# andrewjong/SwapNet

Measured on NVIDIA H100. Metric: images/sec (G+D fwd+bwd) warp-stage 512x512, higher is better.
Workload: dtype fp16/bf16-split x3 tensor-core products, fp32 accumulate (fp32-faithful)

## Files before the change

include/swapnet_b200.h:

```cpp
#ifndef SWAPNET_B200_H
#define SWAPNET_B200_H

#include <stdint.h>

#ifdef __cplusplus
extern "C" {
#endif

#define SN_MAX_TAPS 32
#define SN_MAX_SRC 3

enum { SN_ACT_NONE = 0, SN_ACT_TANH = 1, SN_ACT_LRELU = 2, SN_ACT_RELU = 3 };
enum { SN_LAYOUT_NCHW = 0, SN_LAYOUT_NHWC = 1, SN_LAYOUT_LABEL_U8 = 2, SN_LAYOUT_MASK_I32 = 3 };
#define SN_FMT_BF16 0
#define SN_FMT_F16 1

const char* sn_version(void);
const char* sn_last_error(void);
long long sn_launch_count(void);
void sn_count_replayed(long long n);

typedef struct sn_tap {
  int c_off;
  int kb_off;
// ... 43 lines not shown
  int ksplit;
  int nsplit;
  int deterministic;
} sn_wgrad_desc;

typedef struct sn_plan sn_plan;

int sn_tap_gemm_plan_create(const sn_tap_gemm_desc* desc, sn_plan** out);
int sn_wgrad_plan_create(const sn_wgrad_desc* desc, sn_plan** out);
int sn_plan_run(const sn_plan* plan, void* stream);
void sn_plan_destroy(sn_plan* plan);
int sn_plan_has_stats(const sn_plan* plan);
int sn_plan_geometry(const sn_plan* plan, int* out);
long long sn_plan_workspace_bytes(const sn_plan* plan);
int sn_wgrad_ksplit(const sn_wgrad_desc* desc, int sm_count);

int sn_pack_planes(const float* src, int src_layout, int src_pitch, int n, int c, int h, int w,
                   void* dst_hi, void* dst_lo, int dst_pitch, int dst_coff, int fmt, void* stream);

int sn_pack_concat(int lead, const float* src0, int layout0, int pitch0, int c0, const float* src1, int layout1,
                   int pitch1, int c1, int n, int h, int w, int c_fill, void* dst_hi, void* dst_lo, void* dst2_hi,
                   void* dst2_lo, int dst_pitch, int dst_coff, int fmt, int fmt2, void* stream);

typedef struct sn_scale_item { const float* w; long long count; float* scale2; } sn_scale_item;
typedef struct sn_pack_item {
  const float* src; long long s_row, s_k;
  int rows, taps, taps_pitch, k_real, k_pad, fmt;
  void* hi; void* lo; const float* scale2;
  int slot[16];
  int block_begin;
// ... 224 lines not shown
```

swapnet_b200/_lib.py:

```python
from __future__ import annotations

import ctypes as C
import os

_HERE = os.path.dirname(os.path.abspath(__file__))
LIB_PATH = os.path.join(_HERE, "libswapnet_b200.so")

SN_MAX_TAPS = 32
SN_MAX_SRC = 3
ACT_NONE, ACT_TANH, ACT_LRELU, ACT_RELU = 0, 1, 2, 3
LAYOUT_NCHW, LAYOUT_NHWC, LAYOUT_LABEL_U8, LAYOUT_MASK_I32 = 0, 1, 2, 3
FMT_BF16, FMT_F16 = 0, 1
AUG_NONE, AUG_HFLIP, AUG_VFLIP, AUG_AFFINE_NEAREST, AUG_PERSPECTIVE_BILINEAR = 0, 1, 2, 3, 4
AUG_MAX_OPS = 8


class SnTap(C.Structure):
    _fields_ = [("c_off", C.c_int), ("kb_off", C.c_int), ("dw", C.c_int), ("dh", C.c_int), ("hp", C.c_int)]


class SnTapGemmDesc(C.Structure):
    _fields_ = [
        ("a_hi", C.c_void_p), ("a_lo", C.c_void_p),
        ("a_n", C.c_int), ("a_h", C.c_int), ("a_w", C.c_int), ("a_c", C.c_int), ("a_pitch", C.c_int),
# ... 100 lines not shown

_VP, _I, _LL, _F, _ULL = C.c_void_p, C.c_int, C.c_longlong, C.c_float, C.c_ulonglong
SIGNATURES = {
    "sn_version": (C.c_char_p, []),
    "sn_last_error": (C.c_char_p, []),
    "sn_launch_count": (_LL, []),
    "sn_count_replayed": (None, [_LL]),
    "sn_tap_gemm_plan_create": (_I, [C.POINTER(SnTapGemmDesc), C.POINTER(_VP)]),
    "sn_wgrad_plan_create": (_I, [C.POINTER(SnWgradDesc), C.POINTER(_VP)]),
    "sn_plan_run": (_I, [_VP, _VP]),
    "sn_plan_destroy": (None, [_VP]),
    "sn_plan_has_stats": (_I, [_VP]),
    "sn_plan_geometry": (_I, [_VP, C.POINTER(C.c_int)]),
    "sn_plan_workspace_bytes": (_LL, [_VP]),
    "sn_wgrad_ksplit": (_I, [C.POINTER(SnWgradDesc), _I]),
    "sn_det_slots": (_LL, [_I, _I]),
    "sn_plane_sums_det": (_I, [_VP, _I, _I, _I, _I, _VP, _VP, _LL, _VP]),
    "sn_plane_stats_det": (_I, [_VP, _I, _I, _I, _I, _F, _VP, _VP, _LL, _VP]),
    "sn_bias_grad_det": (_I, [_VP, _VP, _I, _I, _I, _LL, _I, _VP, _VP, _VP, _LL, _VP]),
    "sn_ce_tanh_bwd_det": (_I, [_VP, _I, _VP, _I, C.POINTER(SnGradSrc), _I, _I, _I, _I, _I, _F, _VP, _VP, _VP, _I, _I,
                                _I, _VP, _LL, _VP]),
    "sn_gan_loss_fwd_bwd_det": (_I, [_I, _VP, _LL, _I, _F, _F, _VP, _F, _VP, _VP, _VP, _LL, _VP]),
    "sn_l1_loss_fwd_bwd_det": (_I, [_VP, _I, _VP, _I, _I, _I, _I, _F, _VP, _VP, _I, _VP, _LL, _VP]),
    "sn_to_one_wgrad_det": (_I, [_VP, _VP, _I, _I, _I, _I, _I, _I, _VP, _VP, _I, _I, _I, _I, _VP, _VP, _LL, _VP]),
    "sn_to_one_wgrad_det_slots": (_LL, [_I]),
    "sn_stats_finalize": (_I, [_VP, _I, _I, _F, _VP]),
    "sn_plane_sums": (_I, [_VP, _I, _I, _I, _I, _VP, _VP]),
    "sn_bn_finalize": (_I, [_VP, _I, _I, _I, _I, _F, _F, _VP, _VP, _VP, _VP]),
    "sn_bn_eval_stats": (_I, [_VP, _I, _I, _VP, _VP, _F, _VP]),
    "sn_bn_group_sums": (_I, [_VP, _I, _I, _I, _I, _VP, _VP]),
# ... 91 lines not shown
```

swapnet_b200/csrc/api.cu:

```cuda
#include <stdarg.h>
#include <atomic>
#include "common.cuh"
#include "plan.h"

static thread_local char g_err[1024] = "";
std::atomic<long long> g_launches{0};

void sn_set_error(const char* fmt, ...) {
  va_list ap;
  va_start(ap, fmt);
  vsnprintf(g_err, sizeof(g_err), fmt, ap);
  va_end(ap);
}
void sn_count_launch(int n) { g_launches.fetch_add(n, std::memory_order_relaxed); }

struct sn_plan {
  int kind;
  TapGemmPlan tg;
  WgradPlan wg;
};

static int g_sm_count = 0;
static int sm_count() {
  if (!g_sm_count) {
// ... 53 lines not shown
  out[0] = plan->kind;
  out[1] = (int)g.x;
  out[2] = (int)g.y;
  out[3] = (int)g.z;
  out[4] = plan->kind == 0 ? plan->tg.p.block_n : plan->wg.p.block_n;
  out[5] = plan->kind == 0 ? plan->tg.p.a_chunk : plan->wg.p.y_chunk;
  return SN_OK;
}

long long sn_plan_workspace_bytes(const sn_plan* plan) {
  return plan && plan->kind == 1 ? (long long)plan->wg.ws_bytes : 0;
}

int sn_wgrad_ksplit(const sn_wgrad_desc* desc, int sm_count) { return sn_wgrad_plan_ksplit(desc, sm_count); }

void sn_plan_destroy(sn_plan* plan) {
  if (plan && plan->kind == 0 && plan->tg.p.tile_counter) cudaFree(plan->tg.p.tile_counter);
  if (plan && plan->kind == 1 && plan->wg.p.det_ws) cudaFree(plan->wg.p.det_ws);
  delete plan;
}

}
```

swapnet_b200/csrc/common.cuh:

```cuda
#pragma once
#include <cuda_runtime.h>
#include <cuda.h>
#include <cuda_bf16.h>
#include <cuda_fp16.h>
#include <stdint.h>
#include <stdio.h>
#include <string.h>

void sn_set_error(const char* fmt, ...);
#define SN_OK 0
#define SN_ERR_INVALID (-1)
#define SN_ERR_CUDA (-2)
#define SN_ERR_UNSUPPORTED (-3)
#define SN_NUM_SMS 132
#ifndef SN_FMT_BF16
#define SN_FMT_BF16 0
#define SN_FMT_F16 1
#endif

#define SN_CHECK_CUDA(expr)                                                        \
  do {                                                                             \
    cudaError_t _e = (expr);                                                       \
    if (_e != cudaSuccess) {                                                       \
      sn_set_error("%s:%d CUDA error %s: %s", __FILE__, __LINE__, #expr,           \
// ... 203 lines not shown
        "{\n.reg .pred p;\nsetp.ne.b32 p, %66, 0;\n"
        "wgmma.mma_async.sync.aligned.m64n128k16.f32.bf16.bf16 "
        "{%0, %1, %2, %3, %4, %5, %6, %7, %8, %9, %10, %11, %12, %13, %14, %15, %16, %17, %18, %19, %20, %21, %22, %23, %24, %25, %26, %27, %28, %29, %30, %31, %32, %33, %34, %35, %36, %37, %38, %39, %40, %41, %42, %43, %44, %45, %46, %47, %48, %49, %50, %51, %52, %53, %54, %55, %56, %57, %58, %59, %60, %61, %62, %63}, %64, %65, p, 1, 1, %67, %68;\n}\n"
        : "+f"(d[0]), "+f"(d[1]), "+f"(d[2]), "+f"(d[3]), "+f"(d[4]), "+f"(d[5]), "+f"(d[6]), "+f"(d[7]), "+f"(d[8]), "+f"(d[9]), "+f"(d[10]), "+f"(d[11]), "+f"(d[12]), "+f"(d[13]), "+f"(d[14]), "+f"(d[15]), "+f"(d[16]), "+f"(d[17]), "+f"(d[18]), "+f"(d[19]), "+f"(d[20]), "+f"(d[21]), "+f"(d[22]), "+f"(d[23]), "+f"(d[24]), "+f"(d[25]), "+f"(d[26]), "+f"(d[27]), "+f"(d[28]), "+f"(d[29]), "+f"(d[30]), "+f"(d[31]), "+f"(d[32]), "+f"(d[33]), "+f"(d[34]), "+f"(d[35]), "+f"(d[36]), "+f"(d[37]), "+f"(d[38]), "+f"(d[39]), "+f"(d[40]), "+f"(d[41]), "+f"(d[42]), "+f"(d[43]), "+f"(d[44]), "+f"(d[45]), "+f"(d[46]), "+f"(d[47]), "+f"(d[48]), "+f"(d[49]), "+f"(d[50]), "+f"(d[51]), "+f"(d[52]), "+f"(d[53]), "+f"(d[54]), "+f"(d[55]), "+f"(d[56]), "+f"(d[57]), "+f"(d[58]), "+f"(d[59]), "+f"(d[60]), "+f"(d[61]), "+f"(d[62]), "+f"(d[63])
        : "l"(a), "l"(b), "r"(scale_d), "n"(TA), "n"(TB));
  }
};
template <> struct Wgmma<128, true> {
  template <int TA, int TB>
  static __device__ __forceinline__ void mma(float (&d)[64], uint64_t a, uint64_t b, int scale_d) {
    asm volatile(
        "{\n.reg .pred p;\nsetp.ne.b32 p, %66, 0;\n"
        "wgmma.mma_async.sync.aligned.m64n128k16.f32.f16.f16 "
        "{%0, %1, %2, %3, %4, %5, %6, %7, %8, %9, %10, %11, %12, %13, %14, %15, %16, %17, %18, %19, %20, %21, %22, %23, %24, %25, %26, %27, %28, %29, %30, %31, %32, %33, %34, %35, %36, %37, %38, %39, %40, %41, %42, %43, %44, %45, %46, %47, %48, %49, %50, %51, %52, %53, %54, %55, %56, %57, %58, %59, %60, %61, %62, %63}, %64, %65, p, 1, 1, %67, %68;\n}\n"
        : "+f"(d[0]), "+f"(d[1]), "+f"(d[2]), "+f"(d[3]), "+f"(d[4]), "+f"(d[5]), "+f"(d[6]), "+f"(d[7]), "+f"(d[8]), "+f"(d[9]), "+f"(d[10]), "+f"(d[11]), "+f"(d[12]), "+f"(d[13]), "+f"(d[14]), "+f"(d[15]), "+f"(d[16]), "+f"(d[17]), "+f"(d[18]), "+f"(d[19]), "+f"(d[20]), "+f"(d[21]), "+f"(d[22]), "+f"(d[23]), "+f"(d[24]), "+f"(d[25]), "+f"(d[26]), "+f"(d[27]), "+f"(d[28]), "+f"(d[29]), "+f"(d[30]), "+f"(d[31]), "+f"(d[32]), "+f"(d[33]), "+f"(d[34]), "+f"(d[35]), "+f"(d[36]), "+f"(d[37]), "+f"(d[38]), "+f"(d[39]), "+f"(d[40]), "+f"(d[41]), "+f"(d[42]), "+f"(d[43]), "+f"(d[44]), "+f"(d[45]), "+f"(d[46]), "+f"(d[47]), "+f"(d[48]), "+f"(d[49]), "+f"(d[50]), "+f"(d[51]), "+f"(d[52]), "+f"(d[53]), "+f"(d[54]), "+f"(d[55]), "+f"(d[56]), "+f"(d[57]), "+f"(d[58]), "+f"(d[59]), "+f"(d[60]), "+f"(d[61]), "+f"(d[62]), "+f"(d[63])
        : "l"(a), "l"(b), "r"(scale_d), "n"(TA), "n"(TB));
  }
};


__device__ __forceinline__ uint64_t gmma_smem_desc(uint32_t smem_addr, uint32_t lbo_bytes, uint32_t sbo_bytes,
                                                   uint32_t layout = 1) {
  uint64_t d = 0;
  d |= (uint64_t)((smem_addr >> 4) & 0x3FFF);
  d |= (uint64_t)((lbo_bytes >> 4) & 0x3FFF) << 16;
  d |= (uint64_t)((sbo_bytes >> 4) & 0x3FFF) << 32;
  d |= (uint64_t)(layout & 3u) << 62;
  return d;
}
__host__ __device__ __forceinline__ uint32_t gmma_layout_of_chunk(int chunk) {
// ... 46 lines not shown
```

swapnet_b200/csrc/gemm_tc.cu:

```cuda
#include "common.cuh"
#include "plan.h"

namespace {

constexpr int kBlockM = 128;
constexpr int kTileRing = 4;
constexpr int kTileBytes = 16384;
constexpr int kConsumerWarps = 8;
constexpr int kProducerWarp = kConsumerWarps;
constexpr int kThreads = (kConsumerWarps + 1) * 32;

template <int NSPLIT>
struct Cfg {
  static constexpr int kPlanes = NSPLIT == 3 ? 2 : 1;
  static constexpr int kStages = NSPLIT == 3 ? 3 : 6;
  static constexpr int kStageBytes = kPlanes * 2 * kTileBytes;
  static constexpr int kSmemBytes = kStages * kStageBytes + 1024;
};

__device__ __forceinline__ float apply_act(float v, int act) {
  if (act == SN_ACT_TANH) return tanhf(v);
  return v;
}

__device__ __forceinline__ float quad_col_sum(float v) {
  v += __shfl_xor_sync(0xffffffffu, v, 4);
  v += __shfl_xor_sync(0xffffffffu, v, 8);
  v += __shfl_xor_sync(0xffffffffu, v, 16);
  return v;
}

template <int NSPLIT, int CW, int BN, bool F16>
__global__ void __launch_bounds__(kThreads, 1)
tap_gemm_kernel(const __grid_constant__ TapGemmParams p, const int m_tiles, const int n_tiles, const int total_tiles) {
  const auto tile_coords = [&](int tile, int& mt, int& nt, int& z) {
    nt = tile % n_tiles;
    const int rest = tile / n_tiles;
    mt = rest % m_tiles;
    z = rest / m_tiles;
  };
  using C = Cfg<NSPLIT>;
  extern __shared__ uint8_t smem_raw[];
  __shared__ __align__(8) uint64_t full_bar[C::kStages];
  __shared__ __align__(8) uint64_t empty_bar[C::kStages];
  __shared__ __align__(8) uint64_t tr_full[kTileRing];
  __shared__ __align__(8) uint64_t tr_empty[kTileRing];
  __shared__ int tile_ring[kTileRing];

  const uint32_t smem_base = (smem_u32(smem_raw) + 1023u) & ~1023u;
  uint8_t* smem = smem_raw + (smem_base - smem_u32(smem_raw));
  const int warp = threadIdx.x >> 5;
  const int lane = threadIdx.x & 31;

  constexpr int cw = CW;
  constexpr int tps = 64 / cw;
  const int tpp = p.ntaps / p.nphase;
// ... 47 lines not shown
            const int ch = k - t * p.chunks;
            const TapDesc tap = p.taps[tap0 + t];
            if (p.a_merged) {
              tma_load_5d(&p.tmA[0], &full_bar[s], st, tap.c_off + ch * 64, w0 + tap.dw, h0 + tap.dh, n0, 0);
            } else {
#pragma unroll
              for (int pl = 0; pl < C::kPlanes; ++pl)
                tma_load_5d(&p.tmA[pl], &full_bar[s], st + pl * kTileBytes, tap.c_off + ch * 64,
                            w0 + tap.dw, tap.hp, h0 + tap.dh, n0);
            }
            if (p.b_merged) {
              tma_load_3d(&p.tmB[0], &full_bar[s], st + C::kPlanes * kTileBytes, tap.kb_off + ch * 64, ncol0, 0);
            } else {
#pragma unroll
              for (int pl = 0; pl < C::kPlanes; ++pl)
                tma_load_2d(&p.tmB[pl], &full_bar[s], st + (C::kPlanes + pl) * kTileBytes,
                            tap.kb_off + ch * 64, ncol0);
            }
          } else {
            constexpr int sub = 128 * cw * 2;
#pragma unroll
            for (int j = 0; j < tps; ++j) {
              const TapDesc tap = p.taps[tap0 + k * tps + j];
#pragma unroll
              for (int pl = 0; pl < C::kPlanes; ++pl)
                tma_load_5d(&p.tmA[pl], &full_bar[s], st + pl * kTileBytes + j * sub, tap.c_off,
                            w0 + tap.dw, tap.hp, h0 + tap.dh, n0);
            }
            const int kb = p.taps[tap0 + k * tps].kb_off;
            if (p.b_merged) {
              tma_load_3d(&p.tmB[0], &full_bar[s], st + C::kPlanes * kTileBytes, kb, ncol0, 0);
            } else {
#pragma unroll
              for (int pl = 0; pl < C::kPlanes; ++pl)
                tma_load_2d(&p.tmB[pl], &full_bar[s], st + (C::kPlanes + pl) * kTileBytes, kb, ncol0);
            }
          }
        }
        tile = next;
      }
    }
  } else {
    const int wg = warp >> 2;
    const int quad = lane & 3;
    const int row0 = wg * 64 + (warp & 3) * 16 + (lane >> 2);
    int w_i[2], h_i[2], n_i[2];
#pragma unroll
    for (int h = 0; h < 2; ++h) {
      const int row = row0 + 8 * h;
      w_i[h] = row % p.tw;
      h_i[h] = (row / p.tw) % p.th;
      n_i[h] = row / (p.tw * p.th);
    }
    const float oscale = p.b_scale ? p.b_scale[1] : 1.f;
    float acc[BN / 2];
    uint32_t it = 0;
    for (uint32_t tcount = 0;; ++tcount) {
      const uint32_t slot = tcount % kTileRing, rph = (tcount / kTileRing) & 1;
      mbar_wait(&tr_full[slot], rph);
      const int tile = tile_ring[slot];
      __syncwarp();
      if (lane == 0) mbar_arrive(&tr_empty[slot]);
      if (tile < 0) break;
      for (int k = 0; k < k_iters; ++k, ++it) {
        const uint32_t s = it % C::kStages;
        const uint32_t ph = (it / C::kStages) & 1;
        mbar_wait(&full_bar[s], ph);
        const uint32_t st = smem_base + s * C::kStageBytes;
// ... 17 lines not shown
          }
        }
        wgmma_commit();
        wgmma_wait<0>();
        wgmma_fence_acc(acc);
        if ((threadIdx.x & 127) == 0) mbar_arrive(&empty_bar[s]);
      }

      int mt, nt, z;
      tile_coords(tile, mt, nt, z);
      const int ncol0 = nt * p.block_n;
      const int ph_h = p.nphase == 4 ? (z >> 1) : 0, ph_w = p.nphase == 4 ? (z & 1) : 0;
      int gw[2], gh[2], gn[2];
      bool valid[2];
      float* optr[2];
#pragma unroll
      for (int h = 0; h < 2; ++h) {
        gw[h] = (mt % p.tiles_w) * p.tw + w_i[h];
        gh[h] = ((mt / p.tiles_w) % p.tiles_h) * p.th + h_i[h];
        gn[h] = (mt / (p.tiles_w * p.tiles_h)) * p.nb + n_i[h];
        valid[h] = (row0 + 8 * h < p.a_rows) && (gw[h] < p.m_w) && (gh[h] < p.m_h) && (gn[h] < p.m_n);
        optr[h] = p.out + (long long)gn[h] * p.out_sn + (long long)(gh[h] * p.omh + p.ooh + ph_h) * p.out_sh +
                  (long long)(gw[h] * p.omw + p.oow + ph_w) * p.out_sw + ncol0;
      }
#pragma unroll
      for (int i = 0; i < BN / 8; ++i) {
        const int c = 8 * i + 2 * quad;
        if (BN > 16 && 8 * i >= p.block_n) break;
        if (p.stack_slot) {
#pragma unroll
          for (int h = 0; h < 2; ++h) {
            if (!valid[h]) continue;
#pragma unroll
            for (int e = 0; e < 2; ++e) {
              const int col = ncol0 + c + e;
              const int ph = col / p.stack_slot, ch = col - ph * p.stack_slot;
              if (ph < 4 && ch < p.stack_c) {
                float v = acc[4 * i + 2 * h + e] * oscale;
                if (p.bias) v += p.bias[ch];
                float* o = p.out + (long long)gn[h] * p.out_sn + (long long)(gh[h] * p.omh + (ph >> 1)) * p.out_sh +
                           (long long)(gw[h] * p.omw + (ph & 1)) * p.out_sw + ch;
                *o = apply_act(v, p.act);
              }
            }
// ... 348 lines not shown
      const double eff = (double)useful / (double)(tiles * 128);
      const int rows = w * h * n, perim = w + h, area = w * h;
      const bool better =
          eff > best_eff + 1e-9 ||
          (eff > best_eff - 1e-9 &&
           (rows > best_rows ||
            (rows == best_rows && (area > best_area || (area == best_area && (perim < best_perim || (perim == best_perim && w > *tw)))))));
      if (better) {
        best_eff = eff; best_rows = rows; best_perim = perim; best_area = area;
        *tw = w; *th = h; *nb = n;
      }
    }
  }
}

int sn_tap_gemm_plan_init(TapGemmPlan* plan, const sn_tap_gemm_desc* d) {
  memset(plan, 0, sizeof(*plan));
  TapGemmParams& p = plan->p;
  SN_REQUIRE(d->nsplit == 1 || d->nsplit == 3, "nsplit must be 1 or 3");
  SN_REQUIRE(d->ntaps >= 1 && d->ntaps <= SN_MAX_TAPS, "ntaps out of range: %d", d->ntaps);
  const int a_chunk = d->a_chunk ? d->a_chunk : 64;
  SN_REQUIRE(a_chunk == 64 || a_chunk == 32 || a_chunk == 16, "a_chunk must be 64, 32 or 16");
  if (a_chunk == 64) {
    SN_REQUIRE(d->k_per_tap > 0 && d->k_per_tap % 64 == 0, "k_per_tap must be a multiple of 64");
  } else {
    SN_REQUIRE(d->k_per_tap == a_chunk && d->ntaps % (64 / a_chunk) == 0,
               "narrow operand: k_per_tap must equal a_chunk (%d) and ntaps (%d) be a multiple of %d", a_chunk,
               d->ntaps, 64 / a_chunk);
  }
  p.a_chunk = a_chunk;
  SN_REQUIRE(d->block_n >= 16 && d->block_n <= 128 && d->block_n % 16 == 0,
             "block_n must be a multiple of 16 in [16,128]");
  SN_REQUIRE(d->a_hi && d->b_hi && d->out, "null operand");
  SN_REQUIRE(d->nsplit == 1 || (d->a_lo && d->b_lo), "nsplit=3 needs lo planes");
  SN_REQUIRE(d->a_fmt == d->b_fmt, "A and B of one wgmma must share a 16-bit format (a=%d b=%d)",
             d->a_fmt, d->b_fmt);
  int th, tw, nb;
  pick_patch_conv(d->m_n, d->m_h, d->m_w, &th, &tw, &nb);
  p.a_rows = th * tw * nb;
  p.tw = tw; p.th = th; p.nb = nb;
  p.tiles_w = (d->m_w + tw - 1) / tw;
  p.tiles_h = (d->m_h + th - 1) / th;
  p.tiles_n = (d->m_n + nb - 1) / nb;
  p.m_w = d->m_w; p.m_h = d->m_h; p.m_n = d->m_n;
  p.ntaps = d->ntaps;
  p.chunks = a_chunk == 64 ? d->k_per_tap / 64 : 1;
  for (int t = 0; t < d->ntaps; ++t) {
// ... 33 lines not shown
    p.stats = d->stats;
  plan->stats_bytes = p.stats ? sizeof(double) * 2 * (size_t)d->m_n * d->n_valid : 0;
  p.tile_counter = nullptr;
  SN_CHECK_CUDA(cudaMalloc(&p.tile_counter, 2 * sizeof(int)));
  SN_CHECK_CUDA(cudaMemset(p.tile_counter, 0, 2 * sizeof(int)));
  int rc;
  const void* a_pl[2] = {d->a_hi, d->a_lo};
  const void* b_pl[2] = {d->b_hi, d->b_lo};
  const long long a_ps = d->nsplit == 3 ? (const char*)d->a_lo - (const char*)d->a_hi : 0;
  const long long b_ps = d->nsplit == 3 ? (const char*)d->b_lo - (const char*)d->b_hi : 0;
  p.a_merged = a_chunk == 64 && a_ps > 0 && a_ps % 16 == 0 && p.a_rows % 8 == 0;
  if (p.a_merged && d->a_parity)
    for (int t = 0; t < d->ntaps; ++t) p.taps[t].c_off += p.taps[t].hp * d->a_w * d->a_pitch;
  p.b_merged = b_ps > 0 && b_ps % 16 == 0 && d->block_n % 8 == 0;
  p.a_lo_off = p.a_merged ? p.a_rows * 128 : kTileBytes;
  p.b_lo_off = p.b_merged ? d->block_n * 128 : kTileBytes;
  for (int pl = 0; pl < (d->nsplit == 3 ? 2 : 1); ++pl) {
    if (!(p.a_merged && pl == 1)) {
      rc = sn_make_act_map(&p.tmA[pl], a_pl[pl], d->a_n, d->a_h, d->a_w, d->a_c, d->a_pitch,
                           d->a_parity, tw, th, nb, a_chunk, p.a_merged ? a_ps : 0);
      if (rc) return rc;
    }
    if (!(p.b_merged && pl == 1)) {
      rc = sn_make_weight_map(&p.tmB[pl], b_pl[pl], d->b_rows, d->b_k, d->block_n, p.b_merged ? b_ps : 0);
      if (rc) return rc;
    }
  }
  if (p.a_merged) p.tmA[1] = p.tmA[0];
  if (p.b_merged) p.tmB[1] = p.tmB[0];
  plan->nsplit = d->nsplit;
  plan->grid = dim3(p.tiles_w * p.tiles_h * p.tiles_n, (d->n_valid + d->block_n - 1) / d->block_n, p.nphase);
  return SN_OK;
}

static int mma_n(int block_n) {
  return block_n <= 16 ? 16 : block_n <= 32 ? 32 : block_n <= 64 ? 64 : block_n <= 96 ? 96 : 128;
}

template <int NSPLIT, int CW, int BN, bool F16>
static int launch_tap(const TapGemmPlan* plan, cudaStream_t stream) {
  static bool attr_done = false;
  if (!attr_done) {
    SN_CHECK_CUDA(cudaFuncSetAttribute(tap_gemm_kernel<NSPLIT, CW, BN, F16>, cudaFuncAttributeMaxDynamicSharedMemorySize,
                                       Cfg<NSPLIT>::kSmemBytes));
    attr_done = true;
  }
  static int sms = 0;
  if (sms == 0) {
    int dev = 0;
    SN_CHECK_CUDA(cudaGetDevice(&dev));
    SN_CHECK_CUDA(cudaDeviceGetAttribute(&sms, cudaDevAttrMultiProcessorCount, dev));
  }
  const int m_tiles = (int)plan->grid.x, n_tiles = (int)plan->grid.y;
  const int total = m_tiles * n_tiles * (int)plan->grid.z;
  if (plan->p.stats) SN_CHECK_CUDA(cudaMemsetAsync(plan->p.stats, 0, plan->stats_bytes, stream));
  const int ctas = total < sms ? total : sms;
  tap_gemm_kernel<NSPLIT, CW, BN, F16>
      <<<ctas, kThreads, Cfg<NSPLIT>::kSmemBytes, stream>>>(plan->p, m_tiles, n_tiles, total);
  SN_CHECK_CUDA(cudaGetLastError());
  return SN_OK;
}

template <int NSPLIT, int CW, bool F16>
static int launch_tap_n(const TapGemmPlan* plan, cudaStream_t stream) {
  switch (mma_n(plan->p.block_n)) {
    case 16: return launch_tap<NSPLIT, CW, 16, F16>(plan, stream);
    case 32: return launch_tap<NSPLIT, CW, 32, F16>(plan, stream);
    case 64: return launch_tap<NSPLIT, CW, 64, F16>(plan, stream);
    case 96: return launch_tap<NSPLIT, CW, 96, F16>(plan, stream);
    default: return launch_tap<NSPLIT, CW, 128, F16>(plan, stream);
  }
}

template <int NSPLIT, bool F16>
static int launch_tap_cw(const TapGemmPlan* plan, cudaStream_t stream) {
  const int cw = plan->p.a_chunk;
  if (cw == 64) return launch_tap_n<NSPLIT, 64, F16>(plan, stream);
  if (cw == 32) return launch_tap_n<NSPLIT, 32, F16>(plan, stream);
  return launch_tap_n<NSPLIT, 16, F16>(plan, stream);
}

int sn_tap_gemm_plan_launch(const TapGemmPlan* plan, cudaStream_t stream) {
  const bool f16 = plan->p.a_fmt == SN_FMT_F16;
  if (plan->nsplit == 3) return f16 ? launch_tap_cw<3, true>(plan, stream) : launch_tap_cw<3, false>(plan, stream);
  return f16 ? launch_tap_cw<1, true>(plan, stream) : launch_tap_cw<1, false>(plan, stream);
// ... 177 lines not shown
```

swapnet_b200/csrc/plan.h:

```cpp
#pragma once
#include <cuda.h>
#include <cuda_runtime.h>
#include "../../include/swapnet_b200.h"

struct TapDesc {
  int c_off;
  int kb_off;
  short dw, dh, hp, _pad;
};

struct alignas(64) TapGemmParams {
  CUtensorMap tmA[2];
  CUtensorMap tmB[2];
  TapDesc taps[SN_MAX_TAPS];
  int ntaps, chunks;
  int tiles_w, tiles_h, tiles_n;
  int tw, th, nb;
  int a_rows;
  int m_w, m_h, m_n;
  int block_n, n_valid;
  float* out;
  long long out_sn, out_sh, out_sw;
  int omh, ooh, omw, oow;
  const float* bias;
// ... 35 lines not shown
struct TapGemmPlan {
  TapGemmParams p;
  dim3 grid;
  int nsplit;
  size_t stats_bytes;
};
struct WgradPlan {
  WgradParams p;
  dim3 grid;
  int nsplit;
  size_t ws_bytes;
};

int sn_tap_gemm_plan_init(TapGemmPlan* plan, const sn_tap_gemm_desc* d);
int sn_tap_gemm_plan_launch(const TapGemmPlan* plan, cudaStream_t stream);
int sn_wgrad_plan_init(WgradPlan* plan, const sn_wgrad_desc* d, int sm_count);
int sn_wgrad_plan_launch(const WgradPlan* plan, cudaStream_t stream);
int sn_wgrad_plan_ksplit(const sn_wgrad_desc* d, int sm_count);
```

swapnet_b200/layers.py:

```python
from __future__ import annotations

from typing import List, Optional

import torch

from . import lowering as L
from . import ops
from .ops import ACT_NONE, PackedWeights, Planes


class ConvLayer:
    def __init__(self, kind: str, weight: torch.Tensor, bias: Optional[torch.Tensor], x: Planes, *,
                 nsplit: int = 3, act: int = ACT_NONE, name: str = "", det_ws: Optional[ops.DetWorkspace] = None):
        assert kind in L.KINDS
        self.kind, self.name, self.nsplit, self.act = kind, name, nsplit, act
        self.det_ws = det_ws
        self.weight, self.bias = weight, bias
        self.x = x
        dev = weight.device
        if kind == "convT4s2":
            self.cin, self.cout = weight.shape[0], weight.shape[1]
        else:
            self.cout, self.cin = weight.shape[0], weight.shape[1]
        self.in_h, self.in_w = (x.h - 2, x.w - 2) if kind == "conv3r" else (x.h, x.w)
# ... 37 lines not shown
        self.fused_stats = False
        if y_c_off != 0 or self.act != ACT_NONE:
            stats = None
        if self.stacked:
            d = ops.tap_gemm_desc(self.x, L.head_stacked_spec(self.in_h, self.in_w), self.wp, self.k_pad, y,
                                  4 * L.HEAD_SLOT, bias=self.bias, act=self.act, nsplit=self.nsplit,
                                  block_n=4 * L.HEAD_SLOT, out_c_off=y_c_off, stack_slot=L.HEAD_SLOT, stack_c=self.cout)
            self.fwd_plans.append(ops.tap_gemm_plan(d, keep=(self.x.hi, self.x.lo, self.wp.hi, self.wp.lo, y)))
            self.fwd_plans[-1].tag = ("fwd", self.name)
            return
        specs = L.forward_specs(self.kind, self.in_h, self.in_w)
        merged = ops.merge_phase_specs(specs)
        if merged is not None and (self.k_pad >= 64 or (len(merged.taps) // 4) % (64 // self.k_pad) == 0):
            d = ops.tap_gemm_desc(self.x, merged, self.wp, self.k_pad, y, self.cout, bias=self.bias, act=self.act,
                                  nsplit=self.nsplit, block_n=self.block_n, out_c_off=y_c_off, nphase=4, stats=stats)
            self.fwd_plans.append(ops.tap_gemm_plan(d, keep=(self.x.hi, self.x.lo, self.wp.hi, self.wp.lo, y)))
            self.fwd_plans[-1].tag = ("fwd", self.name)
            self.fused_stats = stats is not None and self.fwd_plans[-1].has_stats
            specs = []
        for spec in specs:
            kw = {}
            if self.kind == "head":
                p = spec.w_phase
                nt = L.head_neff(p >> 1) * L.head_neff(p & 1)
                kw = dict(w_elem_off=self.rows_pad * self.k_pad * L.HEAD_PHASE_OFF[p], w_rows=self.rows_pad,
                          w_k=nt * self.k_pad)
            one = len(specs) == 1 and self.kind != "head"
            d = ops.tap_gemm_desc(self.x, spec, self.wp, self.k_pad, y, self.cout, bias=self.bias,
                                  act=self.act, nsplit=self.nsplit, block_n=self.block_n, out_c_off=y_c_off,
                                  stats=stats if one else None, **kw)
            self.fwd_plans.append(ops.tap_gemm_plan(d, keep=(self.x.hi, self.x.lo, self.wp.hi, self.wp.lo, y)))
            self.fwd_plans[-1].tag = ("fwd", self.name)
            if one:
                self.fused_stats = stats is not None and self.fwd_plans[-1].has_stats

    def register_packs(self, table: "ops.PackTable") -> bool:
        table.add_scale(self.weight, self.wscale)
        if self.kind == "head":
            return True
        table.add_pack(self.weight, self.kind, False, self.k_pad, self.wp)
        if self.wd is not None and self.dgrad_plans:
            table.add_pack(self.weight, self.kind, True, self.dy.c, self.wd)
        return False

    def pack_extra(self) -> None:
# ... 147 lines not shown
```

swapnet_b200/lowering.py:

```python
from __future__ import annotations

from dataclasses import dataclass, field
from typing import List, Tuple

KINDS = ("conv4s2", "convT4s2", "conv3r", "conv4s1", "head", "conv3z")

@dataclass
class Tap:
    pw: int
    kb: int
    dw: int
    dh: int
    hp: int = 0


@dataclass
class GemmSpec:
    parity: bool
    m_h: int
    m_w: int
    taps: List[Tap]
    out_mul: Tuple[int, int] = (1, 1)
    out_off: Tuple[int, int] = (0, 0)
    w_phase: int = 0
# ... 206 lines not shown
    return (co_s, ci_s) if x_is_dy else (ci_s, co_s)


def pad64(c: int) -> int:
    return (c + 63) // 64 * 64


def padc(c: int) -> int:
    if c <= 16:
        return 16
    if c <= 32:
        return 32
    return pad64(c)


def pick_block_n(n_valid: int) -> int:
    if n_valid >= 128:
        return 128
    for b in (16, 32, 64, 128):
        if n_valid <= b:
            return b
    return 128
```

swapnet_b200/ops.py:

```python
from __future__ import annotations

import ctypes as C
from dataclasses import dataclass
from typing import Optional, Sequence, Tuple

import torch

from . import _lib
from . import lowering as L

from ._lib import (ACT_LRELU, ACT_NONE, ACT_RELU, ACT_TANH, FMT_BF16, FMT_F16, LAYOUT_LABEL_U8, LAYOUT_MASK_I32,
                   LAYOUT_NCHW, LAYOUT_NHWC, SnGradSrc, SnNormActBwdDesc, SnNormActDesc, SnTap, SnTapGemmDesc,
                   SnWgradDesc, check)

IN_EPS = 1e-5


def _stream() -> int:
    return torch.cuda.current_stream().cuda_stream


def _ptr(t: Optional[torch.Tensor]) -> Optional[int]:
    return None if t is None else t.data_ptr()

# ... 166 lines not shown
        d.stats = stats.data_ptr()
    return d


def merge_phase_specs(specs) -> Optional[L.GemmSpec]:
    if len(specs) != 4:
        return None
    s0 = specs[0]
    n = len(s0.taps)
    for z, s in enumerate(specs):
        if (s.parity, s.m_h, s.m_w, s.out_mul, s.a_hw, len(s.taps)) != (s0.parity, s0.m_h, s0.m_w, s0.out_mul, s0.a_hw, n):
            return None
        if s.out_off != (z >> 1, z & 1) or s.w_phase != 0:
            return None
    return L.GemmSpec(s0.parity, s0.m_h, s0.m_w, [t for s in specs for t in s.taps], s0.out_mul, (0, 0), 0, s0.a_hw)


def tap_gemm_plan(desc: SnTapGemmDesc, keep: Sequence = ()) -> Plan:
    h = C.c_void_p()
    check(_lib.load().sn_tap_gemm_plan_create(C.byref(desc), C.byref(h)))
    return Plan(h.value, keep)


def tap_gemm_simt(desc: SnTapGemmDesc) -> None:
    check(_lib.load().sn_tap_gemm_simt(C.byref(desc), _stream()))


def wgrad_desc(x: Planes, y: Planes, spec: L.WgradSpec, out: torch.Tensor, s_row: int, s_col: int,
               tap_off: Sequence[int], rows_valid: int, cols_valid: int, *, swap: bool = False,
               nsplit: int = 3, block_n: Optional[int] = None, ksplit: int = 0,
# ... 777 lines not shown
```

Before: 141.2.

## Add 256-wide N tiles for tap GEMM with wide-output 64-channel layers

Adds m64n256k16 wgmma variants and a BN=256 instantiation of the tap GEMM kernel. The stage ring is resized for the larger B tile, with fewer stages to fit shared memory. Forward plans pick BN=256 when A rows are 64-channel, output channels are at least 512, and there are enough tiles for several waves. This raises A-tile reuse and cuts redundant A loads, at the cost of doubled accumulator registers and a shallower pipeline. pick_block_n also now prefers 96 when that pads N less than 128, but forward plans only take the wide choice from it.

```diff
diff --git a/include/swapnet_b200.h b/include/swapnet_b200.h
--- a/include/swapnet_b200.h
+++ b/include/swapnet_b200.h
@@ -81,6 +81,7 @@
 int sn_plan_geometry(const sn_plan* plan, int* out);
 long long sn_plan_workspace_bytes(const sn_plan* plan);
 int sn_wgrad_ksplit(const sn_wgrad_desc* desc, int sm_count);
+int sn_tap_gemm_m_tiles(const sn_tap_gemm_desc* desc);
 
 int sn_pack_planes(const float* src, int src_layout, int src_pitch, int n, int c, int h, int w,
                    void* dst_hi, void* dst_lo, int dst_pitch, int dst_coff, int fmt, void* stream);
diff --git a/swapnet_b200/_lib.py b/swapnet_b200/_lib.py
--- a/swapnet_b200/_lib.py
+++ b/swapnet_b200/_lib.py
@@ -138,6 +138,7 @@
     "sn_plan_geometry": (_I, [_VP, C.POINTER(C.c_int)]),
     "sn_plan_workspace_bytes": (_LL, [_VP]),
     "sn_wgrad_ksplit": (_I, [C.POINTER(SnWgradDesc), _I]),
+    "sn_tap_gemm_m_tiles": (_I, [C.POINTER(SnTapGemmDesc)]),
     "sn_det_slots": (_LL, [_I, _I]),
     "sn_plane_sums_det": (_I, [_VP, _I, _I, _I, _I, _VP, _VP, _LL, _VP]),
     "sn_plane_stats_det": (_I, [_VP, _I, _I, _I, _I, _F, _VP, _VP, _LL, _VP]),
diff --git a/swapnet_b200/csrc/api.cu b/swapnet_b200/csrc/api.cu
--- a/swapnet_b200/csrc/api.cu
+++ b/swapnet_b200/csrc/api.cu
@@ -91,6 +91,8 @@
 
 int sn_wgrad_ksplit(const sn_wgrad_desc* desc, int sm_count) { return sn_wgrad_plan_ksplit(desc, sm_count); }
 
+int sn_tap_gemm_m_tiles(const sn_tap_gemm_desc* desc) { return sn_tap_gemm_plan_m_tiles(desc); }
+
 void sn_plan_destroy(sn_plan* plan) {
   if (plan && plan->kind == 0 && plan->tg.p.tile_counter) cudaFree(plan->tg.p.tile_counter);
   if (plan && plan->kind == 1 && plan->wg.p.det_ws) cudaFree(plan->wg.p.det_ws);
diff --git a/swapnet_b200/csrc/common.cuh b/swapnet_b200/csrc/common.cuh
--- a/swapnet_b200/csrc/common.cuh
+++ b/swapnet_b200/csrc/common.cuh
@@ -241,6 +241,28 @@
         "wgmma.mma_async.sync.aligned.m64n128k16.f32.f16.f16 "
         "{%0, %1, %2, %3, %4, %5, %6, %7, %8, %9, %10, %11, %12, %13, %14, %15, %16, %17, %18, %19, %20, %21, %22, %23, %24, %25, %26, %27, %28, %29, %30, %31, %32, %33, %34, %35, %36, %37, %38, %39, %40, %41, %42, %43, %44, %45, %46, %47, %48, %49, %50, %51, %52, %53, %54, %55, %56, %57, %58, %59, %60, %61, %62, %63}, %64, %65, p, 1, 1, %67, %68;\n}\n"
         : "+f"(d[0]), "+f"(d[1]), "+f"(d[2]), "+f"(d[3]), "+f"(d[4]), "+f"(d[5]), "+f"(d[6]), "+f"(d[7]), "+f"(d[8]), "+f"(d[9]), "+f"(d[10]), "+f"(d[11]), "+f"(d[12]), "+f"(d[13]), "+f"(d[14]), "+f"(d[15]), "+f"(d[16]), "+f"(d[17]), "+f"(d[18]), "+f"(d[19]), "+f"(d[20]), "+f"(d[21]), "+f"(d[22]), "+f"(d[23]), "+f"(d[24]), "+f"(d[25]), "+f"(d[26]), "+f"(d[27]), "+f"(d[28]), "+f"(d[29]), "+f"(d[30]), "+f"(d[31]), "+f"(d[32]), "+f"(d[33]), "+f"(d[34]), "+f"(d[35]), "+f"(d[36]), "+f"(d[37]), "+f"(d[38]), "+f"(d[39]), "+f"(d[40]), "+f"(d[41]), "+f"(d[42]), "+f"(d[43]), "+f"(d[44]), "+f"(d[45]), "+f"(d[46]), "+f"(d[47]), "+f"(d[48]), "+f"(d[49]), "+f"(d[50]), "+f"(d[51]), "+f"(d[52]), "+f"(d[53]), "+f"(d[54]), "+f"(d[55]), "+f"(d[56]), "+f"(d[57]), "+f"(d[58]), "+f"(d[59]), "+f"(d[60]), "+f"(d[61]), "+f"(d[62]), "+f"(d[63])
+        : "l"(a), "l"(b), "r"(scale_d), "n"(TA), "n"(TB));
+  }
+};
+template <> struct Wgmma<256, false> {
+  template <int TA, int TB>
+  static __device__ __forceinline__ void mma(float (&d)[128], uint64_t a, uint64_t b, int scale_d) {
+    asm volatile(
+        "{\n.reg .pred p;\nsetp.ne.b32 p, %130, 0;\n"
+        "wgmma.mma_async.sync.aligned.m64n256k16.f32.bf16.bf16 "
+        "{%0, %1, %2, %3, %4, %5, %6, %7, %8, %9, %10, %11, %12, %13, %14, %15, %16, %17, %18, %19, %20, %21, %22, %23, %24, %25, %26, %27, %28, %29, %30, %31, %32, %33, %34, %35, %36, %37, %38, %39, %40, %41, %42, %43, %44, %45, %46, %47, %48, %49, %50, %51, %52, %53, %54, %55, %56, %57, %58, %59, %60, %61, %62, %63, %64, %65, %66, %67, %68, %69, %70, %71, %72, %73, %74, %75, %76, %77, %78, %79, %80, %81, %82, %83, %84, %85, %86, %87, %88, %89, %90, %91, %92, %93, %94, %95, %96, %97, %98, %99, %100, %101, %102, %103, %104, %105, %106, %107, %108, %109, %110, %111, %112, %113, %114, %115, %116, %117, %118, %119, %120, %121, %122, %123, %124, %125, %126, %127}, %128, %129, p, 1, 1, %131, %132;\n}\n"
+        : "+f"(d[0]), "+f"(d[1]), "+f"(d[2]), "+f"(d[3]), "+f"(d[4]), "+f"(d[5]), "+f"(d[6]), "+f"(d[7]), "+f"(d[8]), "+f"(d[9]), "+f"(d[10]), "+f"(d[11]), "+f"(d[12]), "+f"(d[13]), "+f"(d[14]), "+f"(d[15]), "+f"(d[16]), "+f"(d[17]), "+f"(d[18]), "+f"(d[19]), "+f"(d[20]), "+f"(d[21]), "+f"(d[22]), "+f"(d[23]), "+f"(d[24]), "+f"(d[25]), "+f"(d[26]), "+f"(d[27]), "+f"(d[28]), "+f"(d[29]), "+f"(d[30]), "+f"(d[31]), "+f"(d[32]), "+f"(d[33]), "+f"(d[34]), "+f"(d[35]), "+f"(d[36]), "+f"(d[37]), "+f"(d[38]), "+f"(d[39]), "+f"(d[40]), "+f"(d[41]), "+f"(d[42]), "+f"(d[43]), "+f"(d[44]), "+f"(d[45]), "+f"(d[46]), "+f"(d[47]), "+f"(d[48]), "+f"(d[49]), "+f"(d[50]), "+f"(d[51]), "+f"(d[52]), "+f"(d[53]), "+f"(d[54]), "+f"(d[55]), "+f"(d[56]), "+f"(d[57]), "+f"(d[58]), "+f"(d[59]), "+f"(d[60]), "+f"(d[61]), "+f"(d[62]), "+f"(d[63]), "+f"(d[64]), "+f"(d[65]), "+f"(d[66]), "+f"(d[67]), "+f"(d[68]), "+f"(d[69]), "+f"(d[70]), "+f"(d[71]), "+f"(d[72]), "+f"(d[73]), "+f"(d[74]), "+f"(d[75]), "+f"(d[76]), "+f"(d[77]), "+f"(d[78]), "+f"(d[79]), "+f"(d[80]), "+f"(d[81]), "+f"(d[82]), "+f"(d[83]), "+f"(d[84]), "+f"(d[85]), "+f"(d[86]), "+f"(d[87]), "+f"(d[88]), "+f"(d[89]), "+f"(d[90]), "+f"(d[91]), "+f"(d[92]), "+f"(d[93]), "+f"(d[94]), "+f"(d[95]), "+f"(d[96]), "+f"(d[97]), "+f"(d[98]), "+f"(d[99]), "+f"(d[100]), "+f"(d[101]), "+f"(d[102]), "+f"(d[103]), "+f"(d[104]), "+f"(d[105]), "+f"(d[106]), "+f"(d[107]), "+f"(d[108]), "+f"(d[109]), "+f"(d[110]), "+f"(d[111]), "+f"(d[112]), "+f"(d[113]), "+f"(d[114]), "+f"(d[115]), "+f"(d[116]), "+f"(d[117]), "+f"(d[118]), "+f"(d[119]), "+f"(d[120]), "+f"(d[121]), "+f"(d[122]), "+f"(d[123]), "+f"(d[124]), "+f"(d[125]), "+f"(d[126]), "+f"(d[127])
+        : "l"(a), "l"(b), "r"(scale_d), "n"(TA), "n"(TB));
+  }
+};
+template <> struct Wgmma<256, true> {
+  template <int TA, int TB>
+  static __device__ __forceinline__ void mma(float (&d)[128], uint64_t a, uint64_t b, int scale_d) {
+    asm volatile(
+        "{\n.reg .pred p;\nsetp.ne.b32 p, %130, 0;\n"
+        "wgmma.mma_async.sync.aligned.m64n256k16.f32.f16.f16 "
+        "{%0, %1, %2, %3, %4, %5, %6, %7, %8, %9, %10, %11, %12, %13, %14, %15, %16, %17, %18, %19, %20, %21, %22, %23, %24, %25, %26, %27, %28, %29, %30, %31, %32, %33, %34, %35, %36, %37, %38, %39, %40, %41, %42, %43, %44, %45, %46, %47, %48, %49, %50, %51, %52, %53, %54, %55, %56, %57, %58, %59, %60, %61, %62, %63, %64, %65, %66, %67, %68, %69, %70, %71, %72, %73, %74, %75, %76, %77, %78, %79, %80, %81, %82, %83, %84, %85, %86, %87, %88, %89, %90, %91, %92, %93, %94, %95, %96, %97, %98, %99, %100, %101, %102, %103, %104, %105, %106, %107, %108, %109, %110, %111, %112, %113, %114, %115, %116, %117, %118, %119, %120, %121, %122, %123, %124, %125, %126, %127}, %128, %129, p, 1, 1, %131, %132;\n}\n"
+        : "+f"(d[0]), "+f"(d[1]), "+f"(d[2]), "+f"(d[3]), "+f"(d[4]), "+f"(d[5]), "+f"(d[6]), "+f"(d[7]), "+f"(d[8]), "+f"(d[9]), "+f"(d[10]), "+f"(d[11]), "+f"(d[12]), "+f"(d[13]), "+f"(d[14]), "+f"(d[15]), "+f"(d[16]), "+f"(d[17]), "+f"(d[18]), "+f"(d[19]), "+f"(d[20]), "+f"(d[21]), "+f"(d[22]), "+f"(d[23]), "+f"(d[24]), "+f"(d[25]), "+f"(d[26]), "+f"(d[27]), "+f"(d[28]), "+f"(d[29]), "+f"(d[30]), "+f"(d[31]), "+f"(d[32]), "+f"(d[33]), "+f"(d[34]), "+f"(d[35]), "+f"(d[36]), "+f"(d[37]), "+f"(d[38]), "+f"(d[39]), "+f"(d[40]), "+f"(d[41]), "+f"(d[42]), "+f"(d[43]), "+f"(d[44]), "+f"(d[45]), "+f"(d[46]), "+f"(d[47]), "+f"(d[48]), "+f"(d[49]), "+f"(d[50]), "+f"(d[51]), "+f"(d[52]), "+f"(d[53]), "+f"(d[54]), "+f"(d[55]), "+f"(d[56]), "+f"(d[57]), "+f"(d[58]), "+f"(d[59]), "+f"(d[60]), "+f"(d[61]), "+f"(d[62]), "+f"(d[63]), "+f"(d[64]), "+f"(d[65]), "+f"(d[66]), "+f"(d[67]), "+f"(d[68]), "+f"(d[69]), "+f"(d[70]), "+f"(d[71]), "+f"(d[72]), "+f"(d[73]), "+f"(d[74]), "+f"(d[75]), "+f"(d[76]), "+f"(d[77]), "+f"(d[78]), "+f"(d[79]), "+f"(d[80]), "+f"(d[81]), "+f"(d[82]), "+f"(d[83]), "+f"(d[84]), "+f"(d[85]), "+f"(d[86]), "+f"(d[87]), "+f"(d[88]), "+f"(d[89]), "+f"(d[90]), "+f"(d[91]), "+f"(d[92]), "+f"(d[93]), "+f"(d[94]), "+f"(d[95]), "+f"(d[96]), "+f"(d[97]), "+f"(d[98]), "+f"(d[99]), "+f"(d[100]), "+f"(d[101]), "+f"(d[102]), "+f"(d[103]), "+f"(d[104]), "+f"(d[105]), "+f"(d[106]), "+f"(d[107]), "+f"(d[108]), "+f"(d[109]), "+f"(d[110]), "+f"(d[111]), "+f"(d[112]), "+f"(d[113]), "+f"(d[114]), "+f"(d[115]), "+f"(d[116]), "+f"(d[117]), "+f"(d[118]), "+f"(d[119]), "+f"(d[120]), "+f"(d[121]), "+f"(d[122]), "+f"(d[123]), "+f"(d[124]), "+f"(d[125]), "+f"(d[126]), "+f"(d[127])
         : "l"(a), "l"(b), "r"(scale_d), "n"(TA), "n"(TB));
   }
 };
diff --git a/swapnet_b200/csrc/gemm_tc.cu b/swapnet_b200/csrc/gemm_tc.cu
--- a/swapnet_b200/csrc/gemm_tc.cu
+++ b/swapnet_b200/csrc/gemm_tc.cu
@@ -10,12 +10,14 @@
 constexpr int kProducerWarp = kConsumerWarps;
 constexpr int kThreads = (kConsumerWarps + 1) * 32;
 
-template <int NSPLIT>
+template <int NSPLIT, int BN = 128>
 struct Cfg {
   static constexpr int kPlanes = NSPLIT == 3 ? 2 : 1;
-  static constexpr int kStages = NSPLIT == 3 ? 3 : 6;
-  static constexpr int kStageBytes = kPlanes * 2 * kTileBytes;
+  static constexpr int kBPlaneBytes = BN > 128 ? BN * 128 : kTileBytes;
+  static constexpr int kStages = BN > 128 ? (NSPLIT == 3 ? 2 : 4) : (NSPLIT == 3 ? 3 : 6);
+  static constexpr int kStageBytes = kPlanes * (kTileBytes + kBPlaneBytes);
   static constexpr int kSmemBytes = kStages * kStageBytes + 1024;
+  static_assert(kSmemBytes <= 227 * 1024, "stage ring exceeds the 227 KB of shared memory a CTA can have");
 };
 
 __device__ __forceinline__ float apply_act(float v, int act) {
@@ -39,7 +41,7 @@
     mt = rest % m_tiles;
     z = rest / m_tiles;
   };
-  using C = Cfg<NSPLIT>;
+  using C = Cfg<NSPLIT, BN>;
   extern __shared__ uint8_t smem_raw[];
   __shared__ __align__(8) uint64_t full_bar[C::kStages];
   __shared__ __align__(8) uint64_t empty_bar[C::kStages];
@@ -117,7 +119,7 @@
             } else {
 #pragma unroll
               for (int pl = 0; pl < C::kPlanes; ++pl)
-                tma_load_2d(&p.tmB[pl], &full_bar[s], st + (C::kPlanes + pl) * kTileBytes,
+                tma_load_2d(&p.tmB[pl], &full_bar[s], st + C::kPlanes * kTileBytes + pl * C::kBPlaneBytes,
                             tap.kb_off + ch * 64, ncol0);
             }
           } else {
@@ -136,7 +138,7 @@
             } else {
 #pragma unroll
               for (int pl = 0; pl < C::kPlanes; ++pl)
-                tma_load_2d(&p.tmB[pl], &full_bar[s], st + (C::kPlanes + pl) * kTileBytes, kb, ncol0);
+                tma_load_2d(&p.tmB[pl], &full_bar[s], st + C::kPlanes * kTileBytes + pl * C::kBPlaneBytes, kb, ncol0);
             }
           }
         }
@@ -148,13 +150,16 @@
     const int quad = lane & 3;
     const int row0 = wg * 64 + (warp & 3) * 16 + (lane >> 2);
     int w_i[2], h_i[2], n_i[2];
-#pragma unroll
-    for (int h = 0; h < 2; ++h) {
-      const int row = row0 + 8 * h;
-      w_i[h] = row % p.tw;
-      h_i[h] = (row / p.tw) % p.th;
-      n_i[h] = row / (p.tw * p.th);
-    }
+    const auto patch_rows = [&]() {
+#pragma unroll
+      for (int h = 0; h < 2; ++h) {
+        const int row = row0 + 8 * h;
+        w_i[h] = row % p.tw;
+        h_i[h] = (row / p.tw) % p.th;
+        n_i[h] = row / (p.tw * p.th);
+      }
+    };
+    if (BN <= 128) patch_rows();
     const float oscale = p.b_scale ? p.b_scale[1] : 1.f;
     float acc[BN / 2];
     uint32_t it = 0;
@@ -202,6 +207,7 @@
       int gw[2], gh[2], gn[2];
       bool valid[2];
       float* optr[2];
+      if (BN > 128) patch_rows();
 #pragma unroll
       for (int h = 0; h < 2; ++h) {
         gw[h] = (mt % p.tiles_w) * p.tw + w_i[h];
@@ -215,7 +221,7 @@
       for (int i = 0; i < BN / 8; ++i) {
         const int c = 8 * i + 2 * quad;
         if (BN > 16 && 8 * i >= p.block_n) break;
-        if (p.stack_slot) {
+        if (BN <= 128 && p.stack_slot) {
 #pragma unroll
           for (int h = 0; h < 2; ++h) {
             if (!valid[h]) continue;
@@ -594,6 +600,14 @@
   }
 }
 
+static int mma_n(int block_n) {
+  return block_n <= 16 ? 16 : block_n <= 32 ? 32 : block_n <= 64 ? 64 : block_n <= 96 ? 96 : block_n <= 128 ? 128 : 256;
+}
+
+static int b_plane_bytes(int block_n) {
+  return mma_n(block_n) > 128 ? mma_n(block_n) * 128 : kTileBytes;
+}
+
 int sn_tap_gemm_plan_init(TapGemmPlan* plan, const sn_tap_gemm_desc* d) {
   memset(plan, 0, sizeof(*plan));
   TapGemmParams& p = plan->p;
@@ -609,8 +623,10 @@
                d->ntaps, 64 / a_chunk);
   }
   p.a_chunk = a_chunk;
-  SN_REQUIRE(d->block_n >= 16 && d->block_n <= 128 && d->block_n % 16 == 0,
-             "block_n must be a multiple of 16 in [16,128]");
+  SN_REQUIRE(d->block_n >= 16 && d->block_n <= (a_chunk == 64 ? 256 : 128) && d->block_n % 16 == 0,
+             "block_n must be a multiple of 16 in [16,128], or up to 256 for 64-channel A rows (block_n=%d, a_chunk=%d)",
+             d->block_n, a_chunk);
+  SN_REQUIRE(d->block_n <= 128 || d->stack_slot == 0, "the phase-stacked head takes block_n <= 128");
   SN_REQUIRE(d->a_hi && d->b_hi && d->out, "null operand");
   SN_REQUIRE(d->nsplit == 1 || (d->a_lo && d->b_lo), "nsplit=3 needs lo planes");
   SN_REQUIRE(d->a_fmt == d->b_fmt, "A and B of one wgmma must share a 16-bit format (a=%d b=%d)",
@@ -674,7 +690,7 @@
     for (int t = 0; t < d->ntaps; ++t) p.taps[t].c_off += p.taps[t].hp * d->a_w * d->a_pitch;
   p.b_merged = b_ps > 0 && b_ps % 16 == 0 && d->block_n % 8 == 0;
   p.a_lo_off = p.a_merged ? p.a_rows * 128 : kTileBytes;
-  p.b_lo_off = p.b_merged ? d->block_n * 128 : kTileBytes;
+  p.b_lo_off = p.b_merged ? d->block_n * 128 : b_plane_bytes(d->block_n);
   for (int pl = 0; pl < (d->nsplit == 3 ? 2 : 1); ++pl) {
     if (!(p.a_merged && pl == 1)) {
       rc = sn_make_act_map(&p.tmA[pl], a_pl[pl], d->a_n, d->a_h, d->a_w, d->a_c, d->a_pitch,
@@ -693,8 +709,12 @@
   return SN_OK;
 }
 
-static int mma_n(int block_n) {
-  return block_n <= 16 ? 16 : block_n <= 32 ? 32 : block_n <= 64 ? 64 : block_n <= 96 ? 96 : 128;
+int sn_tap_gemm_plan_m_tiles(const sn_tap_gemm_desc* d) {
+  SN_REQUIRE(d && d->m_n > 0 && d->m_h > 0 && d->m_w > 0, "tap_gemm_m_tiles: bad descriptor");
+  int th, tw, nb;
+  pick_patch_conv(d->m_n, d->m_h, d->m_w, &th, &tw, &nb);
+  const int m_tiles = ((d->m_w + tw - 1) / tw) * ((d->m_h + th - 1) / th) * ((d->m_n + nb - 1) / nb);
+  return m_tiles * (d->nphase == 4 ? 4 : 1);
 }
 
 template <int NSPLIT, int CW, int BN, bool F16>
@@ -702,7 +722,7 @@
   static bool attr_done = false;
   if (!attr_done) {
     SN_CHECK_CUDA(cudaFuncSetAttribute(tap_gemm_kernel<NSPLIT, CW, BN, F16>, cudaFuncAttributeMaxDynamicSharedMemorySize,
-                                       Cfg<NSPLIT>::kSmemBytes));
+                                       Cfg<NSPLIT, BN>::kSmemBytes));
     attr_done = true;
   }
   static int sms = 0;
@@ -716,7 +736,7 @@
   if (plan->p.stats) SN_CHECK_CUDA(cudaMemsetAsync(plan->p.stats, 0, plan->stats_bytes, stream));
   const int ctas = total < sms ? total : sms;
   tap_gemm_kernel<NSPLIT, CW, BN, F16>
-      <<<ctas, kThreads, Cfg<NSPLIT>::kSmemBytes, stream>>>(plan->p, m_tiles, n_tiles, total);
+      <<<ctas, kThreads, Cfg<NSPLIT, BN>::kSmemBytes, stream>>>(plan->p, m_tiles, n_tiles, total);
   SN_CHECK_CUDA(cudaGetLastError());
   return SN_OK;
 }
@@ -728,7 +748,10 @@
     case 32: return launch_tap<NSPLIT, CW, 32, F16>(plan, stream);
     case 64: return launch_tap<NSPLIT, CW, 64, F16>(plan, stream);
     case 96: return launch_tap<NSPLIT, CW, 96, F16>(plan, stream);
-    default: return launch_tap<NSPLIT, CW, 128, F16>(plan, stream);
+    case 128: return launch_tap<NSPLIT, CW, 128, F16>(plan, stream);
+    default:
+      if constexpr (CW == 64) return launch_tap<NSPLIT, CW, 256, F16>(plan, stream);
+      SN_REQUIRE(false, "block_n %d needs 64-channel A rows", plan->p.block_n);
   }
 }
 
diff --git a/swapnet_b200/csrc/plan.h b/swapnet_b200/csrc/plan.h
--- a/swapnet_b200/csrc/plan.h
+++ b/swapnet_b200/csrc/plan.h
@@ -73,6 +73,7 @@
 
 int sn_tap_gemm_plan_init(TapGemmPlan* plan, const sn_tap_gemm_desc* d);
 int sn_tap_gemm_plan_launch(const TapGemmPlan* plan, cudaStream_t stream);
+int sn_tap_gemm_plan_m_tiles(const sn_tap_gemm_desc* d);
 int sn_wgrad_plan_init(WgradPlan* plan, const sn_wgrad_desc* d, int sm_count);
 int sn_wgrad_plan_launch(const WgradPlan* plan, cudaStream_t stream);
 int sn_wgrad_plan_ksplit(const sn_wgrad_desc* d, int sm_count);
diff --git a/swapnet_b200/layers.py b/swapnet_b200/layers.py
--- a/swapnet_b200/layers.py
+++ b/swapnet_b200/layers.py
@@ -75,6 +75,7 @@
         if merged is not None and (self.k_pad >= 64 or (len(merged.taps) // 4) % (64 // self.k_pad) == 0):
             d = ops.tap_gemm_desc(self.x, merged, self.wp, self.k_pad, y, self.cout, bias=self.bias, act=self.act,
                                   nsplit=self.nsplit, block_n=self.block_n, out_c_off=y_c_off, nphase=4, stats=stats)
+            d.block_n = ops.wide_block_n(d)
             self.fwd_plans.append(ops.tap_gemm_plan(d, keep=(self.x.hi, self.x.lo, self.wp.hi, self.wp.lo, y)))
             self.fwd_plans[-1].tag = ("fwd", self.name)
             self.fused_stats = stats is not None and self.fwd_plans[-1].has_stats
@@ -90,6 +91,8 @@
             d = ops.tap_gemm_desc(self.x, spec, self.wp, self.k_pad, y, self.cout, bias=self.bias,
                                   act=self.act, nsplit=self.nsplit, block_n=self.block_n, out_c_off=y_c_off,
                                   stats=stats if one else None, **kw)
+            if self.kind != "head":
+                d.block_n = ops.wide_block_n(d)
             self.fwd_plans.append(ops.tap_gemm_plan(d, keep=(self.x.hi, self.x.lo, self.wp.hi, self.wp.lo, y)))
             self.fwd_plans[-1].tag = ("fwd", self.name)
             if one:
diff --git a/swapnet_b200/lowering.py b/swapnet_b200/lowering.py
--- a/swapnet_b200/lowering.py
+++ b/swapnet_b200/lowering.py
@@ -244,9 +244,14 @@
     return pad64(c)
 
 
-def pick_block_n(n_valid: int) -> int:
+WIDE_MIN_WAVES = 3
+
+
+def pick_block_n(n_valid: int, chunk: int = 0, m_tiles: int = 0, sms: int = 132) -> int:
+    if chunk == 64 and n_valid >= 512 and m_tiles * -(-n_valid // 256) >= WIDE_MIN_WAVES * sms:
+        return 256
     if n_valid >= 128:
-        return 128
+        return 96 if -(-n_valid // 96) * 96 < -(-n_valid // 128) * 128 else 128
     for b in (16, 32, 64, 128):
         if n_valid <= b:
             return b
diff --git a/swapnet_b200/ops.py b/swapnet_b200/ops.py
--- a/swapnet_b200/ops.py
+++ b/swapnet_b200/ops.py
@@ -204,6 +204,18 @@
         if s.out_off != (z >> 1, z & 1) or s.w_phase != 0:
             return None
     return L.GemmSpec(s0.parity, s0.m_h, s0.m_w, [t for s in specs for t in s.taps], s0.out_mul, (0, 0), 0, s0.a_hw)
+
+
+def tap_gemm_m_tiles(desc: SnTapGemmDesc) -> int:
+    n = _lib.load().sn_tap_gemm_m_tiles(C.byref(desc))
+    check(min(n, 0))
+    return n
+
+
+def wide_block_n(desc: SnTapGemmDesc) -> int:
+    sms = torch.cuda.get_device_properties(torch.cuda.current_device()).multi_processor_count
+    bn = L.pick_block_n(desc.n_valid, desc.a_chunk, tap_gemm_m_tiles(desc), sms)
+    return bn if bn == 256 else desc.block_n
 
 
 def tap_gemm_plan(desc: SnTapGemmDesc, keep: Sequence = ()) -> Plan:
```

New measurement: 143.1, median of 6. +1.3%, better.
